# wangchou/whisper.coreml

Measured on AMD Instinct MI355X. Metric: xRT (audio-s/s) large-v3 beam=5 @1/2/4/8 GPU; p50 per-token decode ms, higher is better.
Workload: dtype fp16; 1 GPU; large-v3 beam=5 transcribe() of one 600 s file, 30 s clip grid, condition_on_previous_text=False, temperature=0; model=large-v3, global_batch=20, seq_len=448

## Files before the change

### whisper.coreml_amd/csrc/wh_gemm.h

```cpp
#pragma once
#include "wh_common.h"

namespace wh {

enum Epi {
  EPI_STORE = 0,
  EPI_STORE_GELU = 1,
  EPI_RESID = 2,
  EPI_GELU_POS = 3,
  EPI_HEADSPLIT = 4,
  EPI_QKV_DEC = 5,
  EPI_F32_COLS = 6,
  EPI_PARTIAL = 7,
  EPI_QKV_ENC = 8,
};

struct GemmArgs {
  const void* X = nullptr;
  const void* W = nullptr;
  const float* bias = nullptr;
  int M = 0, N = 0, K = 0;
  int ldx = 0;
  int x_group_rows = 1 << 30;
  int64_t x_group_stride = 0;
// ... 59 lines not shown
  } else if constexpr (EPI == EPI_QKV_ENC) {
    if (n < 2 * a.hs_state) {
      T* o = reinterpret_cast<T*>(a.out) + (int64_t)gi * a.out_group_stride + (int64_t)ri * a.ldo + n;
      store4(o, v[0], v[1], v[2], v[3]);
    } else {
      const int c = n - 2 * a.hs_state, h = c >> 6, d = c & 63;
      const int q = ri & 31;
      const int pt = (ri & ~31) + 8 * ((q & 15) >> 2) + 4 * (q >> 4) + (q & 3);
      T* o = reinterpret_cast<T*>(a.vc) + (((int64_t)gi * a.hs_heads + h) * 64 + d) * a.hs_T + pt;
#pragma unroll
      for (int j = 0; j < 4; ++j) o[(int64_t)j * a.hs_T] = from_f32<T>(v[j]);
    }
  } else if constexpr (EPI == EPI_QKV_DEC) {
    const int ns = a.hs_state;
    if (n < ns) {
      store4(reinterpret_cast<T*>(a.out) + (int64_t)m * a.ldo + n, v[0], v[1], v[2], v[3]);
    } else {
      const int which = n >= 2 * ns;
      const int c = n - ns * (1 + which), h = c >> 6, d = c & 63;
      const int w = a.row_win[m], sl = a.row_slot[m], p = a.row_pos[m];
      const int64_t idx = ((((int64_t)w * a.kv_beams + sl) * a.hs_heads + h) * a.kv_ctx + p) * 64 + d;
      T* base = reinterpret_cast<T*>(which ? a.vc : a.kc);
      store4(base + idx, v[0], v[1], v[2], v[3]);
    }
  }
}

template <typename T, int EPI, int MI, int NI, int MG, typename RowF, typename ColF>
WH_DEV void tile_epilogue(const GemmArgs& a, const float4_t (&acc)[MI][NI], RowF mrow, ColF ncol) {
  static_assert(MI % MG == 0, "row-tile groups");
  constexpr bool LD = EPI == EPI_RESID || EPI == EPI_GELU_POS;
  float4_t bv[NI];
#pragma unroll
  for (int ni = 0; ni < NI; ++ni) bv[ni] = a.bias ? load4f(a.bias + ncol(ni)) : (float4_t){0.f, 0.f, 0.f, 0.f};
#pragma unroll
  for (int g0 = 0; g0 < MI; g0 += MG) {
    float4_t xv[LD ? MG : 1][LD ? NI : 1];
    if constexpr (LD) {
#pragma unroll
      for (int j = 0; j < MG; ++j) {
        const int m = mrow(g0 + j);
        const int gi = m / a.x_group_rows, ri = m - gi * a.x_group_rows;
#pragma unroll
        for (int ni = 0; ni < NI; ++ni) {
          xv[j][ni] = (float4_t){0.f, 0.f, 0.f, 0.f};
          if (m < a.M) {
            if constexpr (EPI == EPI_RESID) xv[j][ni] = load4f(a.out_f32 + (int64_t)m * a.ldo + ncol(ni));
            else xv[j][ni] = load4f(a.pos + (int64_t)ri * a.N + ncol(ni));
          }
        }
      }
    }
#pragma unroll
    for (int j = 0; j < MG; ++j) {
      const int m = mrow(g0 + j);
      if (m >= a.M) continue;
      const int gi = m / a.x_group_rows, ri = m - gi * a.x_group_rows;
#pragma unroll
      for (int ni = 0; ni < NI; ++ni) {
        const int n = ncol(ni);
        float4_t v = acc[g0 + j][ni];
        if (a.bias) v += bv[ni];
        if constexpr (EPI == EPI_RESID) {
          float4_t c = xv[j][ni];
          c += v;
          store4(a.out_f32 + (int64_t)m * a.ldo + n, c[0], c[1], c[2], c[3]);
        } else if constexpr (EPI == EPI_GELU_POS) {
          const float4_t p = xv[j][ni];
          store4(a.out_f32 + (int64_t)m * a.ldo + n, gelu_f(v[0]) + p[0], gelu_f(v[1]) + p[1], gelu_f(v[2]) + p[2],
                 gelu_f(v[3]) + p[3]);
        } else {
          epilogue_store<T, EPI>(a, m, gi, ri, n, v);
        }
      }
    }
  }
}

template <typename T>
int launch_gemm(const GemmArgs& a, int epi, hipStream_t st);
template <typename T>
int launch_gemm_tiles(const GemmArgs& a, int epi, int tile_sel, hipStream_t st);

template <typename T>
int launch_proj_partial(const GemmArgs& a, int max_z, hipStream_t st, int* z_out, hipEvent_t ev0 = nullptr,
                        hipEvent_t ev1 = nullptr);

bool proj1_supported(int R, int n);
template <typename T>
int launch_proj1(const GemmArgs& a, int epi, bool ln, hipStream_t st, hipEvent_t ev0 = nullptr,
                 hipEvent_t ev1 = nullptr);

int gemv_ksplit(int M, int N, int K, int max_z = 16, int mt_block = 0);

}
```

### whisper.coreml_amd/csrc/wh_gemm.hip

```cpp
#include "wh_gemm.h"

#include <algorithm>
#include <type_traits>
#include <cstdlib>

namespace wh {

constexpr int TBM = 128, TBN = 128, TKB = 128;
constexpr int TROW = TKB + 16;

template <typename T, int EPI, int TBN_ = TBN, int KZ = 1>
__global__ __launch_bounds__(256, 2) void k_gemm_tile(GemmArgs a) {
  static_assert(KZ == 1 || KZ == 2, "two K halves at most (their sum commutes)");
  constexpr int BK = TKB / (int)sizeof(T);
  constexpr int KS = BK / 32;
  constexpr int WCH = TBN_ / 32;
  constexpr int NI = TBN_ / 32;
  __shared__ __attribute__((aligned(16))) char smem[2][(TBM + TBN_) * TROW];

  const int ntn = a.N / TBN_;
  const int ntm = (a.M + TBM - 1) / TBM;
  const int rid = xcd_remap(blockIdx.x, ntm * ntn * KZ);
  const int bid = rid / KZ, kz = rid - bid * KZ;
  const int tm = bid / ntn, tn = bid % ntn;
// ... 810 lines not shown
      if (!RAG || c < MT * 16 * CPR) *reinterpret_cast<float4_t*>(xs + (c / CPR) * XS_ROW + (c % CPR) * 16) = xr[i];
    }
    __syncthreads();
    const bool more = kc + KCH < Kc;
    if (more) issue(kc + KCH, wn);
#pragma unroll
    for (int s = 0; s < KS; ++s) {
      if (s < ns) {
#pragma unroll
        for (int mt = 0; mt < MT; ++mt) {
          Frag<T> xf;
          frag_load(xf, reinterpret_cast<const T*>(xs + (mt * 16 + r) * XS_ROW) + s * 32 + 8 * g);
          mfma_step(acc[mt], wf[s], xf);
        }
      }
    }
    __syncthreads();
    if (more) {
#pragma unroll
      for (int s = 0; s < KS; ++s) wf[s] = wn[s];
    }
  }
  const int n = n0 + 4 * g;
#pragma unroll
  for (int mt = 0; mt < MT; ++mt) {
    const int m = mb + mt * 16 + r;
    if (m >= a.M || n >= a.N) continue;
    float4_t v = acc[mt];
    if (EPI == EPI_F32_COLS) {
#if WH_WT
      const auto rs = wt_rsrc(a.out_f32);
#pragma unroll
      for (int j = 0; j < 4; ++j)
        if (n + j < a.N) wt_store1(rs, (m * a.ldo + n + j) * 4, v[j] + (a.bias ? a.bias[n + j] : 0.f));
#else
      float* o = a.out_f32 + (int64_t)m * a.ldo;
#pragma unroll
      for (int j = 0; j < 4; ++j)
        if (n + j < a.N) o[n + j] = v[j] + (a.bias ? a.bias[n + j] : 0.f);
#endif
      continue;
    }
    if (EPI == EPI_PARTIAL) {
#if WH_WT
      wt_store4(wt_rsrc(a.out_f32), (int)((((int64_t)kz * a.M + m) * a.ldo + n) * 4), v);
#else
      store4(a.out_f32 + ((int64_t)kz * a.M + m) * a.ldo + n, v[0], v[1], v[2], v[3]);
#endif
      continue;
    }
    if (a.bias) v += load4f(a.bias + n);
    epilogue_store<T, EPI>(a, m, 0, m, n, v);
  }
}

static int rows_per_block(int M, int mt_block) {
  const int mt = (M + 15) / 16;
  if (mt_block > 0) return std::min(mt_block, std::min(mt, 8));
  return mt >= 8 ? 8 : mt;
}

int gemv_ksplit(int M, int N, int K, int max_z, int mt_block) {
  const char* env = tune_env("WHISPER_HIP_GEMV_WGS");
  const int target = env ? atoi(env) : 256;
  const int mt = (M + 15) / 16;
  const bool xpath = mt >= 3;
  const int rp = rows_per_block(M, mt_block);
  const int wgs = (xpath ? (N + 63) / 64 : (N + 15) / 16) * ((M + 16 * rp - 1) / (16 * rp));
  const int steps = K / 32;
  int best = 1;
  for (int z = 1; z <= 16 && z <= max_z && z <= steps; ++z)
    if (wgs * z <= target) best = z;
  return best;
}

template <typename T>
int launch_gemm_tiles(const GemmArgs& a, int epi, int tile_sel, hipStream_t st);

template <typename T>
int launch_gemm(const GemmArgs& a, int epi, hipStream_t st) {
  return launch_gemm_tiles<T>(a, epi, 256, st);
}

template <typename T>
int launch_gemm_tiles(const GemmArgs& a, int epi, int tile_sel, hipStream_t st) {
  if (a.M <= 0) return 0;
  const bool big = a.M > 128 && (a.N % TBN) == 0 && (a.K % (TKB / (int)sizeof(T))) == 0 && epi != EPI_F32_COLS &&
                   epi != EPI_PARTIAL && a.x_rows == nullptr;
  const bool t256 = big && sizeof(T) == 2 && (tile_sel == 256 || tile_sel == 257) && a.M >= 256 && (a.N % g256::BN) == 0 &&
                    (a.K % (2 * g256::BK)) == 0 && epi != EPI_QKV_DEC &&
                    ((a.M + g256::BM - 1) / g256::BM) * (a.N / g256::BN) >= 256;
  if (t256) {
    const int nwg = ((a.M + g256::BM - 1) / g256::BM) * (a.N / g256::BN);
    switch (epi) {
#define CASE(E)                                                   \
  case E:                                                         \
    if (tile_sel == 257) k_gemm_256<E, 32><<<nwg, 512, 0, st>>>(a), wh_launched("k_gemm_256"); \
    else k_gemm_256<E><<<nwg, 512, 0, st>>>(a), wh_launched("k_gemm_256");                    \
    break;
      CASE(EPI_STORE) CASE(EPI_STORE_GELU) CASE(EPI_RESID) CASE(EPI_GELU_POS) CASE(EPI_HEADSPLIT) CASE(EPI_QKV_ENC)
#undef CASE
      default: return -1;
    }
  } else if (big) {
    const int ntm = (a.M + TBM - 1) / TBM;
    const bool half = ntm * (a.N / TBN) < 256 && (a.N % 64) == 0 && tile_sel != 129;
    const int nwg = ntm * (a.N / (half ? 64 : TBN));
    const bool kz2 = half && sizeof(T) == 2 && (epi == EPI_RESID || epi == EPI_GELU_POS) && a.p1_slab && a.p1_cnt &&
                     (a.K / (TKB / (int)sizeof(T))) % 2 == 0 && (int64_t)nwg * 64 <= a.p1_slabs && tile_sel != 128;
    if (kz2) {
      if (epi == EPI_RESID) k_gemm_tile<T, EPI_RESID, 64, 2><<<2 * nwg, 256, 0, st>>>(a), wh_launched("k_gemm_tile");
      else k_gemm_tile<T, EPI_GELU_POS, 64, 2><<<2 * nwg, 256, 0, st>>>(a), wh_launched("k_gemm_tile");
      return 0;
    }
    switch (epi) {
#define CASE(E)                                                       \
  case E:                                                             \
    if (half) k_gemm_tile<T, E, 64><<<nwg, 256, 0, st>>>(a), wh_launched("k_gemm_tile");          \
    else k_gemm_tile<T, E><<<nwg, 256, 0, st>>>(a), wh_launched("k_gemm_tile");                   \
    break;
      CASE(EPI_STORE) CASE(EPI_STORE_GELU) CASE(EPI_RESID) CASE(EPI_GELU_POS) CASE(EPI_HEADSPLIT) CASE(EPI_QKV_DEC)
      CASE(EPI_QKV_ENC)
#undef CASE
      default: return -1;
    }
  } else {
    if (a.K % 32) return -2;
    if (a.x_group_rows != a.M && a.x_group_rows != 0 && a.x_group_rows < a.M) return -3;
    const int mt = (a.M + 15) / 16;
    const int rows_per = rows_per_block(a.M, a.mt_block);
    const int ks = epi == EPI_PARTIAL ? a.ksplit : 1;
    if (ks < 1 || ks > a.K / 32) return -4;
    static const bool vocab_small = [] {
      const char* e = tune_env("WHISPER_HIP_VOCAB_SMALL");
      return !(e && e[0] == '0');
    }();
    if (a.xf32 && !(vocab_small && epi == EPI_F32_COLS && a.N >= 16384 && a.M <= 8 && a.K <= 1280 && a.K % 32 == 0 &&
                    !a.x_rows))
      return -6;
    static const bool vocab1 = [] {
      const char* e = tune_env("WHISPER_HIP_VOCAB1");
      return !(e && e[0] == '0');
    }();
    if (sizeof(T) == 2 && vocab1 && a.xf32 && a.K == 1280 && !a.bias && a.M <= 8 && (a.N + 15) / 16 <= 256 * 13) {
      constexpr int D = 6;
      const int lds = 8 * (1280 * 2 + 16) + 13 * 8 * 64 * 16;
      static bool attr = hipFuncSetAttribute(reinterpret_cast<const void*>(&k_vocab1<D>),
                                             hipFuncAttributeMaxDynamicSharedMemorySize, 160 * 1024) == hipSuccess;
      if (!attr) return -5;
      k_vocab1<D><<<256, 512, lds, st>>>(a), wh_launched("k_vocab1");
      return 0;
    }
    const int vxrow = a.K * (int)sizeof(T) + 16;
    const int vrg_max = std::min(64, (152 * 1024) / vxrow);
    const int vgrp = (a.M + vrg_max - 1) / vrg_max;
    if (vocab_small && epi == EPI_F32_COLS && !a.bias && a.N >= 16384 && a.M <= (sizeof(T) == 2 ? 32 : 16) && vgrp <= 4 &&
        a.K <= 1280 && a.K % 32 == 0) {
      const int rg = (a.M + vgrp - 1) / vgrp, mtv = (rg + 15) / 16;
      const int lds = rg * vxrow;
      const int grid = vgrp * std::max(1, std::min(256 / vgrp, (a.N + 127) / 128));
      GemmArgs av = a;
      av.row_groups = vgrp;
      auto go = [&](auto mtc) {
        constexpr int MTV = decltype(mtc)::value;
        static bool attr = hipFuncSetAttribute(reinterpret_cast<const void*>(&k_vocab_small<T, MTV>),
                                               hipFuncAttributeMaxDynamicSharedMemorySize, 160 * 1024) == hipSuccess;
// ... 99 lines not shown
```

### whisper.coreml_amd/csrc/wh_runtime.hip

```cpp
#include <hip/hip_runtime.h>

#include <algorithm>
#include <chrono>
#include <cmath>
#include <cstdio>
#include <cstring>
#include <set>
#include <string>
#include <vector>

#include "whisper_hip.h"
#include "wh_align.h"
#include "wh_audio.h"
#include "wh_gemm.h"
#include "wh_host.h"
#include "wh_kernels.h"

using namespace wh;

static thread_local std::string g_release_error;

namespace {

constexpr int CTX = 448;
constexpr int HCTX = CTX + 1;
constexpr int NSPLIT = 8;
static int enc_chunk() {
  static const int v = [] {
    const char* e = tune_env("WHISPER_HIP_ENC_CHUNK");
    const int c = e ? atoi(e) : 16;
    return c >= 1 && c <= 64 ? c : 16;
  }();
  return v;
}
constexpr int PRE_ROWS = 1024;
constexpr int MROWS = 3008;
constexpr int H1ROWS = 3002;
constexpr int KC = 9;
constexpr int EKZ_TILES(int n) { return 12 * (n / 64); }
constexpr int RSPLIT = 16;

struct Arena {
  char* base = nullptr;
  size_t cap = 0, off = 0;
  void* take(size_t bytes) {
    off = (off + 255) & ~size_t(255);
    void* p = base + off;
    off += bytes;
    return off <= cap ? p : nullptr;
  }
};

template <typename T>
struct EncLayer {
  float *ln1_g, *ln1_b, *bqkv, *bo, *ln2_g, *ln2_b, *b1, *b2;
  T *wqkv, *wo, *w1, *w2;
};
template <typename T>
struct DecLayer {
  float *ln1_g, *ln1_b, *bqkv, *bo, *lnx_g, *lnx_b, *bqx, *box, *ln2_g, *ln2_b, *b1, *b2;
  T *wqkv, *wo, *wqx, *wox, *w1, *w2;
  T* wqx_f = nullptr;
};

}

struct wh_ctx {
  virtual std::string step_kernels(int n_win, int group) const = 0;
  virtual ~wh_ctx() {}
  virtual int load(const std::string& name, const float* data, const int64_t* shape, int ndim) = 0;
  virtual int finalize() = 0;
  virtual int encode(int n_win, const int64_t* seeks, const int* segs) = 0;
  virtual int read_xa(int slot, float* out) = 0;
  virtual int read_ckv(int slot, int layer, float* k, float* v) = 0;
  virtual int decode_begin(int n_win, const wh_decode_opts* o, const int* init, const int* n_init, int max_init,
                           const int* sot_index, const int* slots) = 0;
  virtual int decode_steps(int max_steps, int* n_done) = 0;
  virtual int step_prefill(int n_win, int G, const int* init, const int* n_init, int max_init, const int* sot_index,
                           float* lg) = 0;
  virtual int step_tokens(const int* tok, const int* offsets, float* lg) = 0;
  virtual int reorder_kv(const int* src) = 0;
  virtual int decode_read(int slot, int* tokens, float* slp, int* len, int* fin_n, int* fin_tok, int* fin_len,
                          float* fin_score, float* nsp) = 0;
  virtual int prefill_logits(int slot, const int* tokens, int n, float* logits, const int* ah, int na, float* aqk) = 0;
  virtual int align(int slot, const int* tokens, int n, int n_sot, int num_frames, const int* ah, int na, int medfilt,
                    float* probs, int* path, int* plen) = 0;
  virtual int align_batch(int n_win, const int* slots, const int* tokens, const int* n_tokens, int n_sot,
                          const int* num_frames, const int* ah, int na, int medfilt, float* probs, int* paths,
                          int* plens) = 0;
  virtual int dtw(const float* x, int N, int M, int* path, int* plen) = 0;
  virtual int time_stage(int what, int iters, double* ms) = 0;
  virtual int share_weights_from(wh_ctx* src) = 0;
  int sharers = 0;
  wh_ctx* shares_from = nullptr;
  std::vector<float> token_ms;
  double stats[WH_N_STATS] = {0};
  AudioFront audio;
  int n_mels = 0;
  int maxc = 5;
  int maxc_stride = 1;
  int device = 0;
};

namespace {

template <typename T>
struct Ctx : public wh_ctx {
  wh_dims d;
  int ns, nh, La, Ld, V, K1p;
  int Wcap, Gcap;
  hipStream_t st = nullptr;
  Arena wa;
  Arena aa;
  void* wbase = nullptr;
  void* abase = nullptr;
  std::set<std::string> loaded;
// ... 120 lines not shown
    add(n, 4); add(n, 4);
    add((size_t)V * n, sizeof(T)); add(CTX * n, sizeof(T));
    for (int l = 0; l < Ld; ++l) {
      add(n, 4); add(n, 4); add(3 * n * n, sizeof(T)); add(3 * n, 4); add(n * n, sizeof(T)); add(n, 4);
      add(n, 4); add(n, 4); add(n * n, sizeof(T)); add(n, 4); add(n * n, sizeof(T)); add(n, 4);
      add(n, 4); add(n, 4); add(4 * n * n, sizeof(T)); add(4 * n, 4); add(4 * n * n, sizeof(T)); add(n, 4);
    }
    add(n, 4); add(n, 4);
    add(2 * Ld * n * n, sizeof(T)); add(2 * Ld * n, 4);
    const bool wq_frag = xattn_fused_q(n, 1, (int)sizeof(T));
    if (wq_frag)
      for (int l = 0; l < Ld; ++l) add(n * n, sizeof(T));
    HIPCHK(hipMalloc(&wbase, wb));
    HIPCHK(hipMemset(wbase, 0, wb));
    wa.base = (char*)wbase;
    wa.cap = wb;
    auto tk = [&](size_t elems) { return (T*)wa.take(elems * sizeof(T)); };
    auto fk = [&](size_t elems) { return (float*)wa.take(elems * 4); };
    conv1_w = tk(n * K1p); conv1_b = fk(n); conv2_w = tk(n * 3 * n); conv2_b = fk(n); pos_enc = fk(1500 * n);
    enc.resize(La);
    for (auto& e : enc) {
      e.ln1_g = fk(n); e.ln1_b = fk(n); e.wqkv = tk(3 * n * n); e.bqkv = fk(3 * n); e.wo = tk(n * n); e.bo = fk(n);
      e.ln2_g = fk(n); e.ln2_b = fk(n); e.w1 = tk(4 * n * n); e.b1 = fk(4 * n); e.w2 = tk(4 * n * n); e.b2 = fk(n);
    }
    lnp_g = fk(n); lnp_b = fk(n);
    E = tk((size_t)V * n); Pdec = tk(CTX * n);
    dec.resize(Ld);
    for (auto& e : dec) {
      e.ln1_g = fk(n); e.ln1_b = fk(n); e.wqkv = tk(3 * n * n); e.bqkv = fk(3 * n); e.wo = tk(n * n); e.bo = fk(n);
      e.lnx_g = fk(n); e.lnx_b = fk(n); e.wqx = tk(n * n); e.bqx = fk(n); e.wox = tk(n * n); e.box = fk(n);
      e.ln2_g = fk(n); e.ln2_b = fk(n); e.w1 = tk(4 * n * n); e.b1 = fk(4 * n); e.w2 = tk(4 * n * n); e.b2 = fk(n);
    }
    ln_g = fk(n); ln_b = fk(n);
    ckv_w = tk(2 * Ld * n * n); ckv_b = fk(2 * Ld * n);
    if (wq_frag)
      for (auto& e : dec) e.wqx_f = tk(n * n);
    if (!ckv_b || (wq_frag && !dec.back().wqx_f)) return fail(-3, "weight arena overflow");
    expected = 5 + La * 15 + 2 + 2 + Ld * 24 + 2;
    const int WE = std::min(Wcap, enc_chunk());
    PRE = std::max(PRE_ROWS, std::min(Wcap * 240, 8192));
    RD = std::max(Wcap * Gcap, PRE);
    const int LR = std::max(Wcap * Gcap, 2 * Wcap);
    size_t ab = 0;
    auto addA = [&](size_t bytes) { ab += ((bytes + 255) & ~size_t(255)) + 256; };
    addA((size_t)WE * MROWS * n_mels * sizeof(T)); addA((size_t)WE * H1ROWS * n * sizeof(T));
    addA((size_t)WE * 1500 * n * 4); addA((size_t)WE * 1500 * n * sizeof(T)); addA((size_t)WE * 1500 * 3 * n * sizeof(T));
    addA((size_t)WE * 1500 * n * sizeof(T)); addA((size_t)WE * 1500 * 4 * n * sizeof(T));
    addA(((size_t)WE * nh * 64 * TKP + 64) * sizeof(T));
    addA((size_t)Wcap * 1500 * n * sizeof(T));
    addA((size_t)2 * Ld * Wcap * TKP * n * sizeof(T) + 65536);
    if ((int64_t)Wcap * Gcap * CTX * n * (int64_t)sizeof(T) >= ((int64_t)1 << 31) - 4096)
      return fail(-3, "self-KV cache of one layer exceeds 2 GiB: lower max_windows or max_group");
    for (int l = 0; l < Ld; ++l) { addA((size_t)Wcap * Gcap * CTX * n * sizeof(T)); addA((size_t)Wcap * Gcap * CTX * n * sizeof(T)); }
    addA((size_t)RD * n * 4); addA((size_t)RD * n * sizeof(T)); addA((size_t)RD * n * sizeof(T)); addA((size_t)RD * n * sizeof(T));
    addA((size_t)RD * 4 * n * sizeof(T));
    addA((size_t)RD * nh * NSPLIT * 64 * 4); addA((size_t)RD * nh * NSPLIT * 4); addA((size_t)RD * nh * NSPLIT * 4);
    addA((size_t)LR * V * 4); addA((size_t)2 * Wcap * V * 4); addA(Wcap * 4); addA((size_t)RSPLIT * RD * n * 4);
    for (int i = 0; i < 9; ++i) addA(RD * 4);
    for (int i = 0; i < 5; ++i) addA(RD * 4);
    addA(Ld * nh * 4);
    addA(((V + 31) / 32) * 4);
    addA(Wcap * 8); addA(Wcap * 4);
    addA((size_t)Wcap * Gcap * HCTX * 4); addA((size_t)Wcap * Gcap * CTX * 4);
    addA((size_t)Wcap * CTX * 4);
    for (int i = 0; i < 5; ++i) addA(Wcap * 4);
    addA(Wcap * Gcap * 4);
    addA(Wcap * 16 * 4); addA(Wcap * 16 * 4); addA((size_t)Wcap * 16 * HCTX * 4);
    addA((size_t)Wcap * Gcap * KC * 4); addA((size_t)Wcap * Gcap * KC * 4);
    addA((size_t)Wcap * Gcap * LP_SLICES * LP_REC * 4); addA((size_t)Wcap * Gcap * 4);
    addA((size_t)Wcap * 4);
    addA(64);
    addA(64);
    addA((size_t)P1_SLABS * 256 * 4); addA((size_t)(4 * n / 16) * 4);
    addA((size_t)Wcap * nh * XS_NSP * XREC * 4); addA((size_t)Wcap * nh * 4);
    addA((size_t)8 * n * 4);
    addA((size_t)EKZ_TILES(n) * 65536); addA((size_t)EKZ_TILES(n) * 4 * 4);
    HIPCHK(hipMalloc(&abase, ab));
    HIPCHK(hipMemset(abase, 0, ab));
    aa.base = (char*)abase;
    aa.cap = ab;
    auto ta = [&](size_t elems) { return (T*)aa.take(elems * sizeof(T)); };
    auto fa = [&](size_t elems) { return (float*)aa.take(elems * 4); };
    auto ia = [&](size_t elems) { return (int*)aa.take(elems * 4); };
    melT = ta((size_t)WE * MROWS * n_mels); h1 = ta((size_t)WE * H1ROWS * n);
    x_e = fa((size_t)WE * 1500 * n); xn_e = ta((size_t)WE * 1500 * n); qkv_e = ta((size_t)WE * 1500 * 3 * n);
    att_e = ta((size_t)WE * 1500 * n); hm_e = ta((size_t)WE * 1500 * 4 * n);
    vt_e = ta((size_t)WE * nh * 64 * TKP + 64);
    xa = ta((size_t)Wcap * 1500 * n);
    ckv = ta((size_t)2 * Ld * Wcap * TKP * n + 32768 / sizeof(T));
    kc.resize(Ld); vc.resize(Ld);
    for (int l = 0; l < Ld; ++l) { kc[l] = ta((size_t)Wcap * Gcap * CTX * n); vc[l] = ta((size_t)Wcap * Gcap * CTX * n); }
    x_d = fa((size_t)RD * n); xn_d = ta((size_t)RD * n); q_d = ta((size_t)RD * n); att_d = ta((size_t)RD * n);
    hm_d = ta((size_t)RD * 4 * n);
    po = fa((size_t)RD * nh * NSPLIT * 64); pm = fa((size_t)RD * nh * NSPLIT); pl = fa((size_t)RD * nh * NSPLIT);
    logits = fa((size_t)LR * V); logits2 = fa((size_t)2 * Wcap * V); nsp = fa(Wcap); part = fa((size_t)RSPLIT * RD * n);
    row_tok = ia(RD); row_pos = ia(RD); row_win = ia(RD); row_slot = ia(RD); win_row0 = ia(RD); win_nrows = ia(RD);
    win_slot = ia(RD); rows_in = ia(RD); src_rows = ia(RD);
    st_row_win = ia(RD); st_row_slot = ia(RD); st_win_row0 = ia(RD); st_win_nrows = ia(RD); st_win_slot = ia(RD);
    qk_map = ia(Ld * nh);
    suppress = (unsigned*)ia((V + 31) / 32);
    d_seeks = (int64_t*)aa.take(Wcap * 8); d_segs = ia(Wcap);
    S.hist = ia((size_t)Wcap * Gcap * HCTX); S.anc = ia((size_t)Wcap * Gcap * CTX);
    fp_anc = ia((size_t)Wcap * CTX);
    S.len = ia(Wcap); S.sample_begin = ia(Wcap); S.step = ia(Wcap); S.done = ia(Wcap); S.fin_n = ia(Wcap);
    S.sum_lp = fa(Wcap * Gcap);
    S.fin_score = fa(Wcap * 16); S.fin_len = ia(Wcap * 16); S.fin_tok = ia((size_t)Wcap * 16 * HCTX);
    S.cand_val = fa((size_t)Wcap * Gcap * KC); S.cand_idx = ia((size_t)Wcap * Gcap * KC);
    S.lpart = fa((size_t)Wcap * Gcap * LP_SLICES * LP_REC); S.lp_cnt = ia((size_t)Wcap * Gcap);
    S.lpw_cnt = ia((size_t)Wcap);
    S.seed = (unsigned long long*)aa.take(64);
    p1_slab = fa((size_t)P1_SLABS * 256); p1_cnt = ia(4 * n / 16);
    xs_rec = fa((size_t)Wcap * nh * XS_NSP * XREC); xs_cnt = ia((size_t)Wcap * nh);
    x2_d = fa((size_t)8 * n);
    ekz_slab = fa((size_t)EKZ_TILES(n) * 16384); ekz_cnt = ia((size_t)EKZ_TILES(n) * 4);
    if (!fp_anc || !S.seed || !S.cand_idx || !S.lp_cnt || !S.lpw_cnt || !p1_cnt || !xs_cnt || !x2_d || !ekz_cnt)
      return fail(-3, "activation arena overflow");
    S.nw = Wcap; S.G = 1; S.ctx = CTX; S.hctx = HCTX; S.maxc = 16;
    return audio.init(st, stats);
  }

  int up(void* dst, const std::vector<T>& h) {
    HIPCHK(hipMemcpy(dst, h.data(), h.size() * sizeof(T), hipMemcpyHostToDevice));
    return 0;
  }
  int upf(float* dst, const float* src, size_t cnt, float scale = 1.f) {
    if (scale == 1.f) {
      HIPCHK(hipMemcpy(dst, src, cnt * 4, hipMemcpyHostToDevice));
      return 0;
    }
    std::vector<float> t(src, src + cnt);
    for (auto& v : t) v *= scale;
    HIPCHK(hipMemcpy(dst, t.data(), cnt * 4, hipMemcpyHostToDevice));
    return 0;
  }
  int upT(T* dst, const float* src, size_t cnt, float scale = 1.f) {
    std::vector<T> t(cnt);
    for (size_t i = 0; i < cnt; ++i) t[i] = (T)(src[i] * scale);
    return up(dst, t);
  }

  int load(const std::string& name, const float* data, const int64_t* shape, int ndim) override {
    auto need = [&](std::initializer_list<int64_t> want) -> int {
      if ((int)want.size() != ndim) return fail(-4, name + ": bad rank");
      int i = 0;
      for (auto w : want)
        if (shape[i++] != w) return fail(-4, name + ": bad shape");
      return 0;
    };
    const size_t n = ns;
    const float kscale = 0.125f;
    int rc = 0;
    if (name == "encoder.conv1.weight") {
      TRY(need({(int64_t)n, n_mels, 3}));
      std::vector<float> t(n * K1p, 0.f);
      for (size_t o = 0; o < n; ++o)
        for (int c = 0; c < n_mels; ++c)
          for (int j = 0; j < 3; ++j) t[o * K1p + j * n_mels + c] = data[(o * n_mels + c) * 3 + j];
      rc = upT(conv1_w, t.data(), t.size());
    } else if (name == "encoder.conv1.bias") { TRY(need({(int64_t)n})); rc = upf(conv1_b, data, n); }
    else if (name == "encoder.conv2.weight") {
      TRY(need({(int64_t)n, (int64_t)n, 3}));
      std::vector<float> t(n * 3 * n);
      for (size_t o = 0; o < n; ++o)
        for (size_t c = 0; c < n; ++c)
          for (int j = 0; j < 3; ++j) t[o * 3 * n + j * n + c] = data[(o * n + c) * 3 + j];
      rc = upT(conv2_w, t.data(), t.size());
    } else if (name == "encoder.conv2.bias") { TRY(need({(int64_t)n})); rc = upf(conv2_b, data, n); }
    else if (name == "encoder.positional_embedding") { TRY(need({1500, (int64_t)n})); rc = upf(pos_enc, data, 1500 * n); }
    else if (name == "encoder.ln_post.weight") { TRY(need({(int64_t)n})); rc = upf(lnp_g, data, n); }
    else if (name == "encoder.ln_post.bias") { TRY(need({(int64_t)n})); rc = upf(lnp_b, data, n); }
    else if (name == "decoder.token_embedding.weight") { TRY(need({V, (int64_t)n})); rc = upT(E, data, (size_t)V * n); }
    else if (name == "decoder.positional_embedding") { TRY(need({CTX, (int64_t)n})); rc = upT(Pdec, data, CTX * n); }
    else if (name == "decoder.ln.weight") { TRY(need({(int64_t)n})); rc = upf(ln_g, data, n); }
    else if (name == "decoder.ln.bias") { TRY(need({(int64_t)n})); rc = upf(ln_b, data, n); }
    else {
      int l = -1;
      char part[128];
      const bool is_enc = sscanf(name.c_str(), "encoder.blocks.%d.%127s", &l, part) == 2;
      const bool is_dec = !is_enc && sscanf(name.c_str(), "decoder.blocks.%d.%127s", &l, part) == 2;
      if (!is_enc && !is_dec) return fail(-5, "unknown tensor " + name);
      const std::string p(part);
      if (is_enc) {
        if (l < 0 || l >= La) return fail(-5, "layer out of range " + name);
        auto& e = enc[l];
        if (p == "attn.query.weight") { TRY(need({(int64_t)n, (int64_t)n})); rc = upT(e.wqkv, data, n * n); }
        else if (p == "attn.query.bias") { TRY(need({(int64_t)n})); rc = upf(e.bqkv, data, n); }
        else if (p == "attn.key.weight") { TRY(need({(int64_t)n, (int64_t)n})); rc = upT(e.wqkv + n * n, data, n * n, kscale); }
        else if (p == "attn.value.weight") { TRY(need({(int64_t)n, (int64_t)n})); rc = upT(e.wqkv + 2 * n * n, data, n * n); }
        else if (p == "attn.value.bias") { TRY(need({(int64_t)n})); rc = upf(e.bqkv + 2 * n, data, n); }
        else if (p == "attn.out.weight") { TRY(need({(int64_t)n, (int64_t)n})); rc = upT(e.wo, data, n * n); }
        else if (p == "attn.out.bias") { TRY(need({(int64_t)n})); rc = upf(e.bo, data, n); }
        else if (p == "attn_ln.weight") { TRY(need({(int64_t)n})); rc = upf(e.ln1_g, data, n); }
        else if (p == "attn_ln.bias") { TRY(need({(int64_t)n})); rc = upf(e.ln1_b, data, n); }
        else if (p == "mlp_ln.weight") { TRY(need({(int64_t)n})); rc = upf(e.ln2_g, data, n); }
        else if (p == "mlp_ln.bias") { TRY(need({(int64_t)n})); rc = upf(e.ln2_b, data, n); }
        else if (p == "mlp.0.weight") { TRY(need({4 * (int64_t)n, (int64_t)n})); rc = upT(e.w1, data, 4 * n * n); }
        else if (p == "mlp.0.bias") { TRY(need({4 * (int64_t)n})); rc = upf(e.b1, data, 4 * n); }
        else if (p == "mlp.2.weight") { TRY(need({(int64_t)n, 4 * (int64_t)n})); rc = upT(e.w2, data, 4 * n * n); }
        else if (p == "mlp.2.bias") { TRY(need({(int64_t)n})); rc = upf(e.b2, data, n); }
        else return fail(-5, "unknown tensor " + name);
      } else {
        if (l < 0 || l >= Ld) return fail(-5, "layer out of range " + name);
        auto& e = dec[l];
        T* ck = ckv_w + (size_t)(2 * l) * n * n;
        if (p == "attn.query.weight") { TRY(need({(int64_t)n, (int64_t)n})); rc = upT(e.wqkv, data, n * n, kscale); }
        else if (p == "attn.query.bias") { TRY(need({(int64_t)n})); rc = upf(e.bqkv, data, n, kscale); }
        else if (p == "attn.key.weight") { TRY(need({(int64_t)n, (int64_t)n})); rc = upT(e.wqkv + n * n, data, n * n); }
        else if (p == "attn.value.weight") { TRY(need({(int64_t)n, (int64_t)n})); rc = upT(e.wqkv + 2 * n * n, data, n * n); }
        else if (p == "attn.value.bias") { TRY(need({(int64_t)n})); rc = upf(e.bqkv + 2 * n, data, n); }
        else if (p == "attn.out.weight") { TRY(need({(int64_t)n, (int64_t)n})); rc = upT(e.wo, data, n * n); }
        else if (p == "attn.out.bias") { TRY(need({(int64_t)n})); rc = upf(e.bo, data, n); }
        else if (p == "attn_ln.weight") { TRY(need({(int64_t)n})); rc = upf(e.ln1_g, data, n); }
        else if (p == "attn_ln.bias") { TRY(need({(int64_t)n})); rc = upf(e.ln1_b, data, n); }
        else if (p == "cross_attn.query.weight") { TRY(need({(int64_t)n, (int64_t)n})); rc = upT(e.wqx, data, n * n, kscale); }
        else if (p == "cross_attn.query.bias") { TRY(need({(int64_t)n})); rc = upf(e.bqx, data, n, kscale); }
        else if (p == "cross_attn.key.weight") { TRY(need({(int64_t)n, (int64_t)n})); rc = upT(ck, data, n * n); }
        else if (p == "cross_attn.value.weight") { TRY(need({(int64_t)n, (int64_t)n})); rc = upT(ck + n * n, data, n * n); }
        else if (p == "cross_attn.value.bias") { TRY(need({(int64_t)n})); rc = upf(ckv_b + (2 * l + 1) * n, data, n); }
        else if (p == "cross_attn.out.weight") { TRY(need({(int64_t)n, (int64_t)n})); rc = upT(e.wox, data, n * n); }
        else if (p == "cross_attn.out.bias") { TRY(need({(int64_t)n})); rc = upf(e.box, data, n); }
        else if (p == "cross_attn_ln.weight") { TRY(need({(int64_t)n})); rc = upf(e.lnx_g, data, n); }
        else if (p == "cross_attn_ln.bias") { TRY(need({(int64_t)n})); rc = upf(e.lnx_b, data, n); }
        else if (p == "mlp_ln.weight") { TRY(need({(int64_t)n})); rc = upf(e.ln2_g, data, n); }
        else if (p == "mlp_ln.bias") { TRY(need({(int64_t)n})); rc = upf(e.ln2_b, data, n); }
        else if (p == "mlp.0.weight") { TRY(need({4 * (int64_t)n, (int64_t)n})); rc = upT(e.w1, data, 4 * n * n); }
        else if (p == "mlp.0.bias") { TRY(need({4 * (int64_t)n})); rc = upf(e.b1, data, 4 * n); }
        else if (p == "mlp.2.weight") { TRY(need({(int64_t)n, 4 * (int64_t)n})); rc = upT(e.w2, data, 4 * n * n); }
        else if (p == "mlp.2.bias") { TRY(need({(int64_t)n})); rc = upf(e.b2, data, n); }
        else return fail(-5, "unknown tensor " + name);
      }
    }
    if (rc) return rc;
    loaded.insert(name);
    return 0;
  }

  int finalize() override {
    if (loaded.size() != expected)
      return fail(-6, "loaded " + std::to_string(loaded.size()) + " of " + std::to_string(expected) + " tensors");
    for (auto& e : dec)
      if (e.wqx_f) launch_wq_frag(e.wqx, e.wqx_f, ns, st);
    HIPCHK(hipStreamSynchronize(st));
    HIPCHK(hipGetLastError());
    HIPCHK(hipDeviceSynchronize());
    finalized = true;
    return 0;
  }

  int gemm(const void* X, int ldx, const T* W, const float* bias, int M, int N, int K, int epi, GemmArgs a) {
    a.X = X; a.ldx = ldx; a.W = W; a.bias = bias; a.M = M; a.N = N; a.K = K;
    if (a.x_group_rows == (1 << 30)) a.x_group_rows = std::max(M, 1);
    const int rc = launch_gemm<T>(a, epi, st);
    if (rc) return fail(-20, "gemm launch failed code " + std::to_string(rc) + " M=" + std::to_string(M) +
                                 " N=" + std::to_string(N) + " K=" + std::to_string(K));
    return 0;
  }

  int encode_chunk(int s0, int we, bool single = false) {
    const int n = ns;
    GemmArgs g;
    const bool kz = single && we == 1 && sizeof(T) == 2 && !(tune_env("WHISPER_HIP_ENC_KZ") && tune_env("WHISPER_HIP_ENC_KZ")[0] == '0');
    auto kz_on = [&](GemmArgs& ga) {
      if (!kz) return;
      ga.p1_slab = ekz_slab;
      ga.p1_cnt = ekz_cnt;
      ga.p1_slabs = EKZ_TILES(n) * 64;
    };
    const MelView mel = audio.mel();
    launch_mel_windows<T>(mel.p, mel.frames, n_mels, d_seeks + s0, d_segs + s0, melT, (int64_t)MROWS * n_mels, MROWS, we, st);
    g = GemmArgs();
    g.x_group_rows = 3000; g.x_group_stride = (int64_t)MROWS * n_mels;
    g.out = h1; g.ldo = n; g.out_group_stride = (int64_t)H1ROWS * n; g.out_row_off = 1;
    TRY(gemm(melT, n_mels, conv1_w, conv1_b, we * 3000, n, K1p, EPI_STORE_GELU, g));
    launch_zero_rows<T>(h1, (int64_t)H1ROWS * n, n, 0, H1ROWS - 1, we, st);
    g = GemmArgs();
    g.x_group_rows = 1500; g.x_group_stride = (int64_t)H1ROWS * n;
    g.out_f32 = x_e; g.ldo = n; g.pos = pos_enc;
    kz_on(g);
    TRY(gemm(h1, 2 * n, conv2_w, conv2_b, we * 1500, n, 3 * n, EPI_GELU_POS, g));
    const int M = we * 1500;
    for (int l = 0; l < La; ++l) {
      auto& e = enc[l];
      launch_layernorm<T>(x_e, xn_e, e.ln1_g, e.ln1_b, M, n, 1e-7f, nullptr, st);
      g = GemmArgs(); g.out = qkv_e; g.ldo = 3 * n;
      g.x_group_rows = 1500; g.x_group_stride = (int64_t)1500 * n; g.out_group_stride = (int64_t)1500 * 3 * n;
      g.hs_state = n; g.hs_heads = nh; g.hs_T = TKP; g.vc = vt_e;
      TRY(gemm(xn_e, n, e.wqkv, e.bqkv, M, 3 * n, n, EPI_QKV_ENC, g));
      launch_attn_enc<T>(qkv_e, 3 * n, n, nh, 1500, we, (int64_t)1500 * 3 * n, vt_e, TKP, att_e, (int64_t)1500 * n, st);
      g = GemmArgs(); g.out_f32 = x_e; g.ldo = n;
      kz_on(g);
      TRY(gemm(att_e, n, e.wo, e.bo, M, n, n, EPI_RESID, g));
      launch_layernorm<T>(x_e, xn_e, e.ln2_g, e.ln2_b, M, n, 1e-7f, nullptr, st);
      g = GemmArgs(); g.out = hm_e; g.ldo = 4 * n;
      TRY(gemm(xn_e, n, e.w1, e.b1, M, 4 * n, n, EPI_STORE_GELU, g));
      g = GemmArgs(); g.out_f32 = x_e; g.ldo = n;
      kz_on(g);
      TRY(gemm(hm_e, 4 * n, e.w2, e.b2, M, n, 4 * n, EPI_RESID, g));
    }
    T* xa_s = xa + (size_t)s0 * 1500 * n;
    launch_layernorm<T>(x_e, xa_s, lnp_g, lnp_b, M, n, 1e-7f, nullptr, st);
    g = GemmArgs();
    g.x_group_rows = 1500; g.x_group_stride = (int64_t)1500 * n;
    g.out = ckv; g.hs_state = n; g.hs_heads = nh; g.hs_T = TKP; g.hs_nslots = Wcap; g.hs_slot0 = s0;
    TRY(gemm(xa_s, n, ckv_w, ckv_b, M, 2 * Ld * n, n, EPI_HEADSPLIT, g));
    return 0;
  }

  int encode(int n_win, const int64_t* seeks, const int* segs) override {
    if (!finalized) return fail(-9, "weights not finalized");
    if (n_win < 1 || n_win > Wcap) return fail(-9, "n_win out of range");
    const MelView mel = audio.mel();
    if (!mel.p || mel.n_mels != n_mels) return fail(-9, "no mel of the model's n_mels in the context");
    h_seeks.resize(n_win);
    for (int i = 0; i < n_win; ++i) {
      const int64_t s = seeks[i] - mel.f0;
      if (s < 0 || segs[i] < 1 || s + std::min(segs[i], 3000) > mel.frames) return fail(-9, "bad window");
      h_seeks[i] = s;
    }
    TRY(tm.mark(0, st));
    HIPCHK(hipMemcpyAsync(d_seeks, h_seeks.data(), n_win * 8, hipMemcpyHostToDevice, st));
    HIPCHK(hipMemcpyAsync(d_segs, segs, n_win * 4, hipMemcpyHostToDevice, st));
    const int WE = std::min(Wcap, enc_chunk());
    for (int s0 = 0; s0 < n_win; s0 += WE) TRY(encode_chunk(s0, std::min(WE, n_win - s0), n_win == 1));
    TRY(tm.finish(st, stats[WH_STAT_ENCODE_MS]));
    stats[WH_STAT_ENCODE_WINDOWS] += n_win;
    TRY(launch_status(__func__));
    return 0;
  }

  int read_xa(int slot, float* out) override {
    if (slot < 0 || slot >= Wcap) return fail(-10, "slot");
    const size_t cnt = (size_t)1500 * ns;
    std::vector<T> h(cnt);
    HIPCHK(hipMemcpy(h.data(), xa + (size_t)slot * cnt, cnt * sizeof(T), hipMemcpyDeviceToHost));
    for (size_t i = 0; i < cnt; ++i) out[i] = (float)h[i];
    return 0;
  }
  int read_ckv(int slot, int layer, float* k, float* v) override {
    if (slot < 0 || slot >= Wcap || layer < 0 || layer >= Ld) return fail(-10, "slot/layer");
    const size_t per = (size_t)nh * TKP * 64;
    std::vector<T> h(per);
    for (int kv = 0; kv < 2; ++kv) {
      const T* src = ckv + ((size_t)(2 * layer + kv) * Wcap + slot) * per;
      HIPCHK(hipMemcpy(h.data(), src, per * sizeof(T), hipMemcpyDeviceToHost));
      float* o = kv ? v : k;
      for (int hh = 0; hh < nh; ++hh)
        for (int t = 0; t < 1500; ++t) {
          for (int dd = 0; dd < 64; ++dd)
            o[((size_t)hh * 1500 + t) * 64 + dd] =
                kv ? (float)h[(size_t)hh * 64 * TKP + xv_index(dd, t)] : (float)h[((size_t)hh * TKP + t) * 64 + dd];
        }
    }
    return 0;
  }

  int part_slabs(int R, int N) const { return (int)std::min<int64_t>(16, (int64_t)RSPLIT * RD * ns / ((int64_t)R * N)); }

  int slab_h = 0;
  static bool slab16_enabled() {
    static const bool on = [] {
      const char* e = tune_env("WHISPER_HIP_SLAB16");
      return !(e && e[0] == '0');
    }();
    return on;
  }
  static bool slab16_qkv() {
    static const bool on = [] {
      const char* e = tune_env("WHISPER_HIP_SLAB16_QKV");
      return !(e && e[0] == '0');
    }();
    return on;
  }
  int partial(const void* X, int ldx, const T* W, int R, int N, int K, int* ks, bool half_ok = true) {
    GemmArgs g;
    g.X = X; g.ldx = ldx; g.W = W; g.M = R; g.N = N; g.K = K; g.x_group_rows = R;
    g.out_f32 = part; g.ldo = N;
    g.slab_half = half_ok && sizeof(T) == 2 && slab16_enabled();
    slab_h = g.slab_half;
    const int maxz = part_slabs(R, N);
    const bool tev = proj_ev_n < (int)proj_ev.size() / 2;
    const int rc = tev ? launch_proj_partial<T>(g, maxz, st, ks, proj_ev[2 * proj_ev_n], proj_ev[2 * proj_ev_n + 1])
                       : launch_proj_partial<T>(g, maxz, st, ks);
    if (tev && rc == 0) ++proj_ev_n;
    if (rc == 0) return 0;
    if (rc != -1) return fail(-20, "k_proj launch failed code " + std::to_string(rc));
    slab_h = 0;
    *ks = gemv_ksplit(R, N, K, maxz);
    g = GemmArgs();
    g.out_f32 = part; g.ldo = N; g.ksplit = *ks;
    return gemm(X, ldx, W, nullptr, R, N, K, EPI_PARTIAL, g);
  }

  int resid(const T* X, int K, const T* W, const float* b, int R, const float* lg, const float* lb) {
    const int n = ns;
    GemmArgs g;
    if (R > 128) {
      g.out_f32 = x_d; g.ldo = n;
      TRY(gemm(X, K, W, b, R, n, K, EPI_RESID, g));
      launch_resid_ln<T>(x_d, nullptr, 0, 0, nullptr, xn_d, lg, lb, R, n, 1e-5f, st);
    } else {
      int ks = 0;
      TRY(partial(X, K, W, R, n, K, &ks));
      launch_resid_ln<T>(x_d, part, ks, (int64_t)R * n, b, xn_d, lg, lb, R, n, 1e-5f, st, slab_h);
    }
    return 0;
  }
// ... 676 lines not shown
      int max_n = 0;
      for (int i = 0; i < nw; ++i) max_n = std::max(max_n, jobs[w0 + i].N);
      if (launch_dtw_jobs(d_jobs + w0, nw, max_n, jobs[w0].in_lds, lds, -1.f, st))
        return fail(-15, "align: DTW launch");
      HIPCHK(hipStreamSynchronize(st));
      w0 += nw;
    }
    HIPCHK(hipMemcpyAsync(probs, d_probs, prob_off[n_win] * 4, hipMemcpyDeviceToHost, st));
    HIPCHK(hipMemcpyAsync(plens, d_plen, n_win * 4, hipMemcpyDeviceToHost, st));
    HIPCHK(hipMemcpyAsync(paths, d_path, path_off[n_win] * 4, hipMemcpyDeviceToHost, st));
    HIPCHK(hipStreamSynchronize(st));
    TRY(launch_status(__func__));
    return 0;
  }

  int align(int slot, const int* tokens, int n, int n_sot, int num_frames, const int* ah, int na, int medfilt,
            float* probs, int* path, int* plen) override {
    return align_batch(1, &slot, tokens, &n, n_sot, &num_frames, ah, na, medfilt, probs, path, plen);
  }

  int dtw(const float* x, int N, int M, int* path, int* plen) override {
    if (N < 1 || M < 1 || N > 1023 || (int64_t)N * M > (int64_t)1 << 26) return fail(-15, "dtw: shape out of range");
    auto al = [](size_t b) { return (b + 255) & ~size_t(255); };
    const size_t b_x = al((size_t)N * M * 4), b_tr = al(dtw_trace_bytes(N, M)), b_path = al((size_t)2 * (N + M) * 4);
    TRY(ensure_scratch(b_x + b_tr + b_path + 256 + al(sizeof(DtwJob))));
    char* p = scratch.p;
    float* d_x = (float*)p; p += b_x;
    unsigned* d_tr = (unsigned*)p; p += b_tr;
    int* d_path = (int*)p; p += b_path;
    int* d_plen = (int*)p; p += 256;
    DtwJob* d_job = (DtwJob*)p;
    DtwJob job{d_x, d_tr, d_path, d_plen, N, M, 0};
    size_t lds = 0;
    if (dtw_prepare(&job, 1, &lds)) return fail(-15, "dtw: shape");
    HIPCHK(hipMemcpyAsync(d_x, x, (size_t)N * M * 4, hipMemcpyHostToDevice, st));
    HIPCHK(hipMemcpyAsync(d_job, &job, sizeof(job), hipMemcpyHostToDevice, st));
    if (launch_dtw_jobs(d_job, 1, N, job.in_lds, lds, 1.f, st)) return fail(-15, "dtw launch");
    HIPCHK(hipMemcpyAsync(plen, d_plen, 4, hipMemcpyDeviceToHost, st));
    HIPCHK(hipMemcpyAsync(path, d_path, (size_t)2 * (N + M) * 4, hipMemcpyDeviceToHost, st));
    HIPCHK(hipStreamSynchronize(st));
    TRY(launch_status(__func__));
    return 0;
  }

  int prefill_logits(int slot, const int* tokens, int n, float* lg, const int* ah, int na, float* aqk) override {
    float* d_aqk = nullptr;
    float* out = nullptr;
    if (na > 0 && aqk) HIPCHK(hipMalloc((void**)&d_aqk, (size_t)na * n * 1500 * 4));
    HIPCHK(hipMalloc((void**)&out, (size_t)n * V * 4));
    std::vector<std::vector<int>> keep;
    int rc = first_pass(slot, tokens, n, ah, na, d_aqk, keep);
    std::vector<int> s2(n);
    for (int i = 0; i < n; ++i) s2[i] = i;
    for (int r0 = 0; r0 < n && rc == 0; r0 += 128) {
      const int rr = std::min(128, n - r0);
      if (hipMemcpyAsync(rows_in, s2.data() + r0, rr * 4, hipMemcpyHostToDevice, st) != hipSuccess) rc = -100;
      if (!rc) rc = vocab(rows_in, rr, out + (size_t)r0 * V);
      if (!rc && hipStreamSynchronize(st) != hipSuccess) rc = -100;
    }
    if (!rc && hipMemcpyAsync(lg, out, (size_t)n * V * 4, hipMemcpyDeviceToHost, st) != hipSuccess) rc = -100;
    if (!rc && d_aqk && hipMemcpyAsync(aqk, d_aqk, (size_t)na * n * 1500 * 4, hipMemcpyDeviceToHost, st) != hipSuccess)
      rc = -100;
    if (hipStreamSynchronize(st) != hipSuccess && !rc) rc = -100;
    if (hipFree(out) != hipSuccess && !rc) rc = -100;
    if (d_aqk && hipFree(d_aqk) != hipSuccess && !rc) rc = -100;
    if (rc == -100) return fail(-100, "prefill_logits: HIP copy / sync / free failed");
    if (rc) return rc;
    TRY(launch_status(__func__));
    return 0;
  }

  int time_stage(int what, int iters, double* ms) override {
    restore_rows();
    if (what != 0 && what != 7) rows_dirty = true;
    if (what == 0) {
      if (cur_nwin < 1) return fail(-16, "no decode batch");
      if (!eager()) TRY(ensure_graph());
      HIPCHK(hipEventRecord(tm.ev[0], st));
      for (int i = 0; i < iters; ++i) TRY(launch_step());
      HIPCHK(hipEventRecord(tm.ev[1], st));
    } else if (what == 1) {
      HIPCHK(hipEventRecord(tm.ev[0], st));
      for (int i = 0; i < iters; ++i) TRY(encode_chunk(0, 1, true));
      HIPCHK(hipEventRecord(tm.ev[1], st));
    } else if (what == 2 || what == 3 || what == 5 || what == 6) {
      if (cur_nwin < 1) return fail(-16, "no decode batch");
      const bool warm = what >= 5;
      if (warm) what -= 3;
      const int nl = warm ? 1 : Ld;
      const int R = cur_nwin * cur_G, n = ns;
      int launches = 0;
      HIPCHK(hipEventRecord(tm.ev[0], st));
      for (int i = 0; i < iters * (warm ? Ld : 1); ++i)
        for (int l = 0; l < nl; ++l) {
          auto& e = dec[l];
          if (what == 2) {
            TRY(layer_projections(l, R));
            launches += 6;
          } else {
            const T* ck = ckv + (size_t)(2 * l) * Wcap * TKP * n;
            const T* cv = ckv + (size_t)(2 * l + 1) * Wcap * TKP * n;
            XQPart xq = step_xq(cur_G);
            if (!p1_active(R, cur_nwin) && xq_proj_active(cur_G)) {
              xq.qx = xn_d; xq.qwf = e.wqx_f; xq.bias = e.bqx;
            }
            launch_cross_attn<T>(q_d, n, ck, cv, 1500, nh, NSPLIT, cur_nwin, st_win_row0, st_win_nrows, st_win_slot,
                                 (int64_t)TKP * n, po, pm, pl, att_d, n, R, nullptr, nullptr, 0, st, xq);
            ++launches;
          }
        }
      HIPCHK(hipEventRecord(tm.ev[1], st));
      HIPCHK(hipStreamSynchronize(st));
      float t = 0;
      HIPCHK(hipEventElapsedTime(&t, tm.ev[0], tm.ev[1]));
      *ms = t / launches;
      return 0;
    } else if (what == 7) {
      if (cur_nwin < 1) return fail(-16, "no decode batch");
      const int per_step = 6 * Ld;
      proj_ev.resize(2 * per_step * iters);
      for (auto& ev : proj_ev) HIPCHK(hipEventCreateWithFlags(&ev, hipEventDisableSystemFence));
      double tot = 0;
      int launches = 0, rc = 0;
      proj_ev_n = 0;
      for (int i = 0; i < iters && rc == 0; ++i) rc = step_body();
      if (rc == 0 && hipStreamSynchronize(st) != hipSuccess) rc = fail(-100, "time_stage(7): sync failed");
      for (int j = 0; rc == 0 && j < proj_ev_n; ++j) {
        float t = 0;
        if (hipEventElapsedTime(&t, proj_ev[2 * j], proj_ev[2 * j + 1]) != hipSuccess)
          rc = fail(-100, "time_stage(7): hipEventElapsedTime failed");
        tot += t;
        ++launches;
      }
      for (auto& ev : proj_ev)
        if (hipEventDestroy(ev) != hipSuccess && rc == 0) rc = fail(-100, "time_stage(7): hipEventDestroy failed");
      proj_ev.clear();
      proj_ev_n = 0;
      if (rc) return rc;
      *ms = launches ? tot / launches : 0.0;
      return 0;
    } else if (what == 8 || what == 9) {
      if (cur_nwin < 1 || cur_G < 1) return fail(-16, "no decode batch");
      if (p1_active(cur_nwin * cur_G, cur_nwin)) return fail(-2, "time_stage(8/9): the single-window step has no k_self_attn_qkv");
      const int R = cur_nwin * cur_G, n = ns;
      const size_t ab = (size_t)Wcap * Gcap * CTX * sizeof(int);
      int* saved = nullptr;
      if (what == 9) {
        HIPCHK(hipMalloc((void**)&saved, ab));
        HIPCHK(hipMemcpyAsync(saved, S.anc, ab, hipMemcpyDeviceToDevice, st));
        HIPCHK(hipMemsetAsync(S.anc, 0, ab, st));
      }
      int rc = 0;
      if (hipEventRecord(tm.ev[0], st) != hipSuccess) rc = fail(-100, "time_stage(8/9): hipEventRecord failed");
      for (int i = 0; rc == 0 && i < iters; ++i)
        for (int l = 0; rc == 0 && l < Ld; ++l)
          if (launch_self_attn_qkv<T>(part, sa_probe_ks, (int64_t)R * 3 * n, dec[l].bqkv, n, kc[l], vc[l], st_row_win,
                                      st_row_slot, row_pos, S.anc, cur_G, Gcap, nh, CTX, att_d, n, R, st, sa_probe_half))
            rc = fail(-20, "time_stage(8/9): self-attention launch refused");
      if (rc == 0 && hipEventRecord(tm.ev[1], st) != hipSuccess) rc = fail(-100, "time_stage(8/9): hipEventRecord failed");
      if (saved) {
        if (hipMemcpyAsync(S.anc, saved, ab, hipMemcpyDeviceToDevice, st) != hipSuccess && rc == 0)
          rc = fail(-100, "time_stage(9): ancestry restore failed");
        if (hipStreamSynchronize(st) != hipSuccess && rc == 0) rc = fail(-100, "time_stage(9): sync failed");
        if (hipFree(saved) != hipSuccess && rc == 0) rc = fail(-100, "time_stage(9): hipFree failed");
      }
      if (rc) return rc;
// ... 212 lines not shown
```

Baseline: 762.1 audio-s/s.

## Balance encoder chunks and split encoder GEMMs by rows to fill CU waves

```diff
diff --git a/whisper.coreml_amd/csrc/wh_gemm.h b/whisper.coreml_amd/csrc/wh_gemm.h
--- a/whisper.coreml_amd/csrc/wh_gemm.h
+++ b/whisper.coreml_amd/csrc/wh_gemm.h
@@ -165,6 +165,8 @@
 template <typename T>
 int launch_gemm_tiles(const GemmArgs& a, int epi, int tile_sel, hipStream_t st);
 
+int gemm_row_split(int M, int N, int K);
+
 template <typename T>
 int launch_proj_partial(const GemmArgs& a, int max_z, hipStream_t st, int* z_out, hipEvent_t ev0 = nullptr,
                         hipEvent_t ev1 = nullptr);
diff --git a/whisper.coreml_amd/csrc/wh_gemm.hip b/whisper.coreml_amd/csrc/wh_gemm.hip
--- a/whisper.coreml_amd/csrc/wh_gemm.hip
+++ b/whisper.coreml_amd/csrc/wh_gemm.hip
@@ -916,6 +916,22 @@
   return launch_gemm_tiles<T>(a, epi, 256, st);
 }
 
+int gemm_row_split(int M, int N, int K) {
+  using namespace g256;
+  static const bool on = [] {
+    const char* e = tune_env("WHISPER_HIP_ROW_SPLIT");
+    return !(e && e[0] == '0');
+  }();
+  if (!on || M < BM || N % BN || K % (2 * BK)) return M;
+  const int ntn = N / BN, ntm = (M + BM - 1) / BM;
+  const int full = ntm * ntn / 256;
+  if (full < 1 || ntm * ntn % 256 == 0) return M;
+  const int tm1 = full * 256 / ntn;
+  const int rest = ntm - tm1;
+  if (tm1 * ntn < 256 || rest * ntn > 128 || M - tm1 * BM <= 128) return M;
+  return tm1 * BM;
+}
+
 template <typename T>
 int launch_gemm_tiles(const GemmArgs& a, int epi, int tile_sel, hipStream_t st) {
   if (a.M <= 0) return 0;
diff --git a/whisper.coreml_amd/csrc/wh_runtime.hip b/whisper.coreml_amd/csrc/wh_runtime.hip
--- a/whisper.coreml_amd/csrc/wh_runtime.hip
+++ b/whisper.coreml_amd/csrc/wh_runtime.hip
@@ -28,10 +28,14 @@
 static int enc_chunk() {
   static const int v = [] {
     const char* e = tune_env("WHISPER_HIP_ENC_CHUNK");
-    const int c = e ? atoi(e) : 16;
-    return c >= 1 && c <= 64 ? c : 16;
+    const int c = e ? atoi(e) : 20;
+    return c >= 1 && c <= 64 ? c : 20;
   }();
   return v;
+}
+static int enc_chunk_len(int n, int i) {
+  const int chunks = (n + enc_chunk() - 1) / enc_chunk();
+  return n / chunks + (i < n % chunks ? 1 : 0);
 }
 constexpr int PRE_ROWS = 1024;
 constexpr int MROWS = 3008;
@@ -318,10 +322,6 @@
     auto ta = [&](size_t elems) { return (T*)aa.take(elems * sizeof(T)); };
     auto fa = [&](size_t elems) { return (float*)aa.take(elems * 4); };
     auto ia = [&](size_t elems) { return (int*)aa.take(elems * 4); };
-    melT = ta((size_t)WE * MROWS * n_mels); h1 = ta((size_t)WE * H1ROWS * n);
-    x_e = fa((size_t)WE * 1500 * n); xn_e = ta((size_t)WE * 1500 * n); qkv_e = ta((size_t)WE * 1500 * 3 * n);
-    att_e = ta((size_t)WE * 1500 * n); hm_e = ta((size_t)WE * 1500 * 4 * n);
-    vt_e = ta((size_t)WE * nh * 64 * TKP + 64);
     xa = ta((size_t)Wcap * 1500 * n);
     ckv = ta((size_t)2 * Ld * Wcap * TKP * n + 32768 / sizeof(T));
     kc.resize(Ld); vc.resize(Ld);
@@ -349,7 +349,11 @@
     xs_rec = fa((size_t)Wcap * nh * XS_NSP * XREC); xs_cnt = ia((size_t)Wcap * nh);
     x2_d = fa((size_t)8 * n);
     ekz_slab = fa((size_t)EKZ_TILES(n) * 16384); ekz_cnt = ia((size_t)EKZ_TILES(n) * 4);
-    if (!fp_anc || !S.seed || !S.cand_idx || !S.lp_cnt || !S.lpw_cnt || !p1_cnt || !xs_cnt || !x2_d || !ekz_cnt)
+    melT = ta((size_t)WE * MROWS * n_mels); h1 = ta((size_t)WE * H1ROWS * n);
+    x_e = fa((size_t)WE * 1500 * n); xn_e = ta((size_t)WE * 1500 * n); qkv_e = ta((size_t)WE * 1500 * 3 * n);
+    att_e = ta((size_t)WE * 1500 * n); hm_e = ta((size_t)WE * 1500 * 4 * n);
+    vt_e = ta((size_t)WE * nh * 64 * TKP + 64);
+    if (!fp_anc || !S.seed || !S.cand_idx || !S.lp_cnt || !S.lpw_cnt || !p1_cnt || !xs_cnt || !x2_d || !ekz_cnt || !vt_e)
       return fail(-3, "activation arena overflow");
     S.nw = Wcap; S.G = 1; S.ctx = CTX; S.hctx = HCTX; S.maxc = 16;
     return audio.init(st, stats);
@@ -492,6 +496,15 @@
     return 0;
   }
 
+  int gemm_rows(const T* X, int K, const T* W, const float* bias, int M, int N, int epi, GemmArgs a) {
+    const int M1 = sizeof(T) == 2 ? gemm_row_split(M, N, K) : M;
+    TRY(gemm(X, K, W, bias, M1, N, K, epi, a));
+    if (M1 == M) return 0;
+    if (a.out) a.out = reinterpret_cast<T*>(a.out) + (size_t)M1 * a.ldo;
+    if (a.out_f32) a.out_f32 += (size_t)M1 * a.ldo;
+    return gemm(X + (size_t)M1 * K, K, W, bias, M - M1, N, K, epi, a);
+  }
+
   int encode_chunk(int s0, int we, bool single = false) {
     const int n = ns;
     GemmArgs g;
@@ -525,13 +538,13 @@
       launch_attn_enc<T>(qkv_e, 3 * n, n, nh, 1500, we, (int64_t)1500 * 3 * n, vt_e, TKP, att_e, (int64_t)1500 * n, st);
       g = GemmArgs(); g.out_f32 = x_e; g.ldo = n;
       kz_on(g);
-      TRY(gemm(att_e, n, e.wo, e.bo, M, n, n, EPI_RESID, g));
+      TRY(gemm_rows(att_e, n, e.wo, e.bo, M, n, EPI_RESID, g));
       launch_layernorm<T>(x_e, xn_e, e.ln2_g, e.ln2_b, M, n, 1e-7f, nullptr, st);
       g = GemmArgs(); g.out = hm_e; g.ldo = 4 * n;
-      TRY(gemm(xn_e, n, e.w1, e.b1, M, 4 * n, n, EPI_STORE_GELU, g));
+      TRY(gemm_rows(xn_e, n, e.w1, e.b1, M, 4 * n, EPI_STORE_GELU, g));
       g = GemmArgs(); g.out_f32 = x_e; g.ldo = n;
       kz_on(g);
-      TRY(gemm(hm_e, 4 * n, e.w2, e.b2, M, n, 4 * n, EPI_RESID, g));
+      TRY(gemm_rows(hm_e, 4 * n, e.w2, e.b2, M, n, EPI_RESID, g));
     }
     T* xa_s = xa + (size_t)s0 * 1500 * n;
     launch_layernorm<T>(x_e, xa_s, lnp_g, lnp_b, M, n, 1e-7f, nullptr, st);
@@ -556,8 +569,8 @@
     TRY(tm.mark(0, st));
     HIPCHK(hipMemcpyAsync(d_seeks, h_seeks.data(), n_win * 8, hipMemcpyHostToDevice, st));
     HIPCHK(hipMemcpyAsync(d_segs, segs, n_win * 4, hipMemcpyHostToDevice, st));
-    const int WE = std::min(Wcap, enc_chunk());
-    for (int s0 = 0; s0 < n_win; s0 += WE) TRY(encode_chunk(s0, std::min(WE, n_win - s0), n_win == 1));
+    for (int s0 = 0, i = 0; s0 < n_win; s0 += enc_chunk_len(n_win, i++))
+      TRY(encode_chunk(s0, enc_chunk_len(n_win, i), n_win == 1));
     TRY(tm.finish(st, stats[WH_STAT_ENCODE_MS]));
     stats[WH_STAT_ENCODE_WINDOWS] += n_win;
     TRY(launch_status(__func__));
@@ -1400,6 +1413,13 @@
     } else if (what == 1) {
       HIPCHK(hipEventRecord(tm.ev[0], st));
       for (int i = 0; i < iters; ++i) TRY(encode_chunk(0, 1, true));
+      HIPCHK(hipEventRecord(tm.ev[1], st));
+    } else if (what == 10) {
+      if (cur_nwin < 1 || (int)h_seeks.size() < cur_nwin) return fail(-16, "no decode batch");
+      HIPCHK(hipEventRecord(tm.ev[0], st));
+      for (int i = 0; i < iters; ++i)
+        for (int s0 = 0, c = 0; s0 < cur_nwin; s0 += enc_chunk_len(cur_nwin, c++))
+          TRY(encode_chunk(s0, enc_chunk_len(cur_nwin, c), cur_nwin == 1));
       HIPCHK(hipEventRecord(tm.ev[1], st));
     } else if (what == 2 || what == 3 || what == 5 || what == 6) {
       if (cur_nwin < 1) return fail(-16, "no decode batch");
```

Result: no change. 765.6 audio-s/s, median of 6 (+0.5%).
